# ZSHCRWY25/3DRVO-MARL-CollisionAvoidance

Hardware: AMD Instinct MI355X
Metric: drone-steps/sec (env.step throughput) (higher is better)
Workload: dtype f64; 1 GPU; BASELINE config 3 env.step: 64 drones x 4096 envs per GPU, nm=10, 0 buildings, map [50.0, 50.0, 10.0], fused step+auto-reset, f32 actions in HBM; envs_per_gpu=4096, drones=64, diag_build=False, cold_all=False, ablate=0, device_error_word=0

## Files before the change

### 3drvo-marl-collisionavoidance_amd/csrc/rvo3d_capi.hip

```cpp
#include "../../include/rvo3d.h"
#include "rvo3d_device.hpp"

#include <atomic>
#include <cmath>
#include <cstdio>
#include <cstdlib>
#include <cstring>
#include <exception>
#include <new>
#include <string>
#include <vector>

using rvo3d::Params;

namespace {
thread_local std::string g_err;

int fail(int code, const std::string& msg) {
  g_err = msg;
  return code;
}
#define HIP_TRY(expr)                                                            \
  do {                                                                           \
    hipError_t _e = (expr);                                                      \
// ... 197 lines not shown
int launch_policy_rnn_tiles(const rvo3d::RnnTilesArgs& A, unsigned grid, hipStream_t s) {
  constexpr int lds = rvo3d::kRnnTilesWaves * H * 128;
  if (int rc = allow_dynamic_lds<rvo3d::policy_rnn_tiles_kernel<H, ND>>(lds)) return rc;
  hipLaunchKernelGGL((rvo3d::policy_rnn_tiles_kernel<H, ND>), dim3(grid), dim3(64 * rvo3d::kRnnTilesWaves), lds, s, A);
  HIP_TRY(hipGetLastError());
  return RVO3D_OK;
}
bool rnn_tiles_shape_ok(int32_t hidden, int32_t in_dim, int32_t state_dim) {
  return (hidden == 64 || hidden == 256) && in_dim == 9 && state_dim >= 1 && state_dim <= 16;
}

std::atomic<uint64_t*> g_step_dev{nullptr};

rvo3d::PolicySampleArgs sample_args(int32_t tanh_out, const float* log_std, float std_factor, uint64_t seed, uint64_t step,
                                    int64_t rows, float* act, float* logp, float* val, float* dbg_mu, float* dbg_raw) {
  rvo3d::PolicySampleArgs S{};
  S.tanh_out = tanh_out; S.log_std = log_std; S.std_factor = std_factor; S.seed = seed; S.step = step;
  S.step_dev = g_step_dev.load();
  S.rows = rows; S.act = act; S.logp = logp; S.val = val; S.dbg_mu = dbg_mu; S.dbg_raw = dbg_raw;
  return S;
}

template <class Args>
int copy_reader(Args& A, const rvo3d_rnn_policy& net) {
  if (!net.w_ih_f || !net.w_hh_f || !net.b_ih_f || !net.b_hh_f || !net.ln_w || !net.ln_b)
    return fail(RVO3D_ERR_INVALID, "null reader weight");
  const bool bi = net.w_ih_r != nullptr;
  if (bi != (net.w_hh_r != nullptr) || bi != (net.b_ih_r != nullptr) || bi != (net.b_hh_r != nullptr))
    return fail(RVO3D_ERR_INVALID, "the reverse direction needs all four of w_ih_r / w_hh_r / b_ih_r / b_hh_r");
  A.w_ih[0] = net.w_ih_f; A.w_hh[0] = net.w_hh_f; A.b_ih[0] = net.b_ih_f; A.b_hh[0] = net.b_hh_f;
  A.w_ih[1] = net.w_ih_r; A.w_hh[1] = net.w_hh_r; A.b_ih[1] = net.b_ih_r; A.b_hh[1] = net.b_hh_r;
  A.ln_w = net.ln_w; A.ln_b = net.ln_b; A.eps = net.ln_eps;
  return RVO3D_OK;
}
template <class Args>
int copy_heads(Args& A, const rvo3d_mlp_weights& pi, const rvo3d_mlp_weights& v, const char* missing) {
  const rvo3d_mlp_weights* n[2] = {&pi, &v};
  for (int i = 0; i < 2; ++i) {
    if (!n[i]->w1 || !n[i]->b1 || !n[i]->w2 || !n[i]->b2 || !n[i]->w3 || !n[i]->b3)
      return fail(RVO3D_ERR_INVALID, missing);
    A.w1[i] = n[i]->w1; A.b1[i] = n[i]->b1; A.w2[i] = n[i]->w2; A.b2[i] = n[i]->b2; A.w3[i] = n[i]->w3; A.b3[i] = n[i]->b3;
  }
  return RVO3D_OK;
}

template <bool X3>
int64_t mlp_net_bytes(int ks1) { return X3 ? rvo3d::mlp_x3_net_bytes(ks1) : rvo3d::mlp_net_bytes(ks1); }

template <bool X3>
int64_t policy_mlp_blob_bytes(int32_t obs_width) {
  if (obs_width < 1 || obs_width > 126) return -1;
  return 2 * mlp_net_bytes<X3>(rvo3d::mlp_ks1(obs_width));
}

template <bool X3>
int policy_mlp_pack(const rvo3d_mlp_weights* pi, const rvo3d_mlp_weights* v, int32_t obs_width, void* blob, void* stream) {
  if (!pi || !v || !blob) return fail(RVO3D_ERR_INVALID, "null pointer");
  if (obs_width < 1 || obs_width > 126) return fail(RVO3D_ERR_INVALID, "obs_width must be 1..126");
  if (reinterpret_cast<uintptr_t>(blob) & 15) return fail(RVO3D_ERR_INVALID, "blob must be 16-byte aligned");
  rvo3d::MlpPackArgs A;
  A.k_in = obs_width; A.ks1 = rvo3d::mlp_ks1(obs_width);
  if (int rc = copy_heads(A, *pi, *v, "null weight pointer")) return rc;
  A.blob = static_cast<unsigned char*>(blob);
  hipLaunchKernelGGL(X3 ? rvo3d::mlp_x3_pack_kernel : rvo3d::mlp_pack_kernel, dim3(64, 2), dim3(256), 0,
                     static_cast<hipStream_t>(stream), A);
  HIP_TRY(hipGetLastError());
  return RVO3D_OK;
}

template <bool X3>
int policy_mlp_sample(const void* blob, int32_t obs_width, const float* obs, int64_t obs_ld, int64_t rows,
                      const int32_t* vo_count, int32_t state_dim, int32_t row_dim, int32_t tanh_out, const float* log_std,
                      float std_factor, uint64_t seed, uint64_t step, float* act, float* logp, float* val, float* dbg_mu,
                      float* dbg_raw, void* stream) {
  if (!blob || !obs || !log_std || !act || !logp || !val) return fail(RVO3D_ERR_INVALID, "null pointer");
  if (obs_width < 1 || obs_width > 126) return fail(RVO3D_ERR_INVALID, "obs_width must be 1..126");
  if (rows < 0 || obs_ld < obs_width) return fail(RVO3D_ERR_INVALID, "rows < 0 or obs_ld < obs_width");
  if (rows > 0 && ((rows - 1) * obs_ld + obs_width) * 4 > (int64_t)0x7fffffff)
    return fail(RVO3D_ERR_INVALID, "the observation array must stay below 2 GiB per call (32-bit buffer offsets): split the rows");
  if (reinterpret_cast<uintptr_t>(obs) & 3) return fail(RVO3D_ERR_INVALID, "obs must be 4-byte aligned");
  if (reinterpret_cast<uintptr_t>(blob) & 15) return fail(RVO3D_ERR_INVALID, "blob must be 16-byte aligned");
  if (rows == 0) return RVO3D_OK;
  int dev = 0, cus = 0;
  HIP_TRY(hipGetDevice(&dev));
  HIP_TRY(hipDeviceGetAttribute(&cus, hipDeviceAttributeMultiprocessorCount, dev));
  const int ks1 = rvo3d::mlp_ks1(obs_width);
  rvo3d::PolicyMlpArgs A;
  A.blob = static_cast<const unsigned char*>(blob); A.net_bytes = mlp_net_bytes<X3>(ks1);
  A.obs = obs; A.ld_obs = obs_ld; A.k_in = obs_width;
  A.cnt = vo_count; A.state_dim = state_dim; A.row_dim = row_dim;
  if (vo_count && (state_dim < 0 || row_dim < 1 || state_dim > obs_width))
    return fail(RVO3D_ERR_INVALID, "vo_count needs 0 <= state_dim <= obs_width and row_dim >= 1");
  A.S = sample_args(tanh_out, log_std, std_factor, seed, step, rows, act, logp, val, dbg_mu, dbg_raw);
  const int64_t nchunks = (rows + 63) / 64;
  int64_t G = (nchunks + kMlpWaves - 1) / kMlpWaves;
  const int64_t Gmax = cus >= 2 ? cus / 2 : 1;
  if (G > Gmax) G = Gmax;
  const unsigned grid = (unsigned)(2 * G);
  hipStream_t s = static_cast<hipStream_t>(stream);
  switch (ks1) {
    case 1: return launch_policy_mlp<X3, 1>(A, grid, s);
    case 2: return launch_policy_mlp<X3, 2>(A, grid, s);
    case 3: return launch_policy_mlp<X3, 3>(A, grid, s);
    case 4: return launch_policy_mlp<X3, 4>(A, grid, s);
    case 5: return launch_policy_mlp<X3, 5>(A, grid, s);
    case 6: return launch_policy_mlp<X3, 6>(A, grid, s);
    case 7: return launch_policy_mlp<X3, 7>(A, grid, s);
    default: return launch_policy_mlp<X3, 8>(A, grid, s);
  }
}
}

extern "C" {

int rvo3d_version(void) { return RVO3D_VERSION; }
const char* rvo3d_last_error(void) { return g_err.c_str(); }

int rvo3d_create(const rvo3d_config* cfg, rvo3d_env** out) {
  RVO3D_API_BEGIN
  if (!cfg || !out) return fail(RVO3D_ERR_INVALID, "null argument");
  *out = nullptr;
  if (cfg->num_envs < 1 || cfg->num_drones < 1 || cfg->num_drones > rvo3d::kMaxThreads)
    return fail(RVO3D_ERR_INVALID, "need num_envs >= 1 and 1 <= num_drones <= 512");
  if (cfg->max_points < 2 || cfg->num_buildings < 0 || cfg->neighbors_num < 0)
    return fail(RVO3D_ERR_INVALID, "need max_points >= 2, num_buildings >= 0, neighbors_num >= 0");
  if ((long long)cfg->num_envs * cfg->num_drones > (1ll << 30))
    return fail(RVO3D_ERR_INVALID, "num_envs * num_drones too large");
  if (cfg->action_decimals > 9) return fail(RVO3D_ERR_INVALID, "action_decimals must be <= 9");
  DeviceGuard dg;
  if (int rc0 = dg.enter(cfg->device)) return rc0;

  rvo3d_env* h = new (std::nothrow) rvo3d_env();
  if (!h) return fail(RVO3D_ERR_INVALID, "out of host memory");
  struct Owner {
    rvo3d_env* p;
    ~Owner() {
      if (!p) return;
      if (p->arena) (void)hipFree(p->arena);
      delete p;
    }
  } owner{h};
  h->cfg = *cfg;
  Params& P = h->P;
  rvo3d::Cold& C = h->cold;
  std::memset(&P, 0, sizeof P);
  std::memset(&C, 0, sizeof C);
  P.E = cfg->num_envs; P.N = cfg->num_drones; P.P = cfg->max_points;
  C.nb = cfg->num_buildings; P.nm = cfg->neighbors_num; P.env_train = cfg->env_train ? 1 : 0;
  P.W = 12 + 9 * P.nm;
#ifdef RVO3D_DIAG
  if (const char* ab = std::getenv("RVO3D_ABLATE")) P.ablate = std::atoi(ab);
#endif
  C.act_scale = cfg->action_decimals >= 0 ? std::pow(10.0, cfg->action_decimals) : 0.0;
  for (int k = 0; k < 3; ++k) C.map[k] = cfg->map_size[k];
  P.T10 = sq_threshold(10.0);
  C.T5 = sq_threshold(5.0);
  C.bgx = C.bgy = 0; C.bg_inv = 0.0;
  if (cfg->num_buildings > 0 && cfg->map_size[0] > 0 && cfg->map_size[1] > 0 &&
      std::isfinite(cfg->map_size[0]) && std::isfinite(cfg->map_size[1])) {
    const double cs = std::fmax(8.0, std::fmax(cfg->map_size[0], cfg->map_size[1]) / 64.0);
    C.bgx = (int)std::ceil(cfg->map_size[0] / cs); C.bgy = (int)std::ceil(cfg->map_size[1] / cs);
    if (C.bgx < 1) C.bgx = 1;
    if (C.bgy < 1) C.bgy = 1;
    C.bg_inv = 1.0 / cs;
  }
  C.T04 = sq_threshold(0.4);
  {
    double mx = std::fmax(C.map[0], std::fmax(C.map[1], C.map[2]));
    if (!(mx > 0)) mx = 1.0;
    for (int k = 0; k < 3; ++k) C.cen[k] = 0.5 * C.map[k];
    const double cmax = 0.75 * mx + 16.0;
    const double u = std::ldexp(1.0, -24);
    const double eD = u * (2.0 * cmax + 21.0);
    const double band = 2.0 * (2.0 * 1.7320508 * 10.5 * eD + 3.0 * eD * eD + 8.0 * u * 110.25);
    C.cmax = (float)cmax;
    P.band = std::nextafter((float)band, INFINITY);
    const float t10f = std::nextafter((float)(P.T10 + band), INFINITY);
    P.t10n = -std::nextafter(t10f, INFINITY);
    P.bandn = P.band + P.t10n;
    C.kdot = std::nextafter((float)(2.0 * (eD + 4.0 * u * 10.5) * 1.001), INFINITY);
    const double gap = 512.0 * band;
    const double cs = 4.0 * (1.7320508 * eD / std::sqrt(gap) + 8.0 * u);
    P.x1_gap = (float)gap;
    P.x1_k2 = (float)(1.0 - (4e-3 + 4.0 * cs));
    const double cs_out = cs > 1e-3 ? cs : 1e-3;
    P.x1_cs2 = (float)(cs_out * cs_out);
  }

  const int N = P.N;
  int nw = (N + 63) / 64;
  P.nw = nw <= 4 ? nw : 8;
  int epb = P.nw == 1 ? 64 / N : 1;
  if (epb > P.E) epb = P.E;
  const int ring = (P.nw >= 2 && P.nw <= 4) ? 64 * P.nw : N;
  const int threads = P.nw == 1 ? 64 : (int)align_up((size_t)ring, 64);
  size_t lds = rvo3d::lds_bytes(threads, P.nm, epb, ring, P.nw);
#ifdef RVO3D_DIAG
  if (const char* pad = std::getenv("RVO3D_LDS_PAD")) lds += (size_t)std::atoi(pad);
#endif
  if (lds > 160 * 1024) {
    return fail(RVO3D_ERR_INVALID, "neighbors_num * num_drones needs more than 160 KiB of LDS");
  }
  P.epb = epb;
  C.zf_div = (uint32_t)((P.W & 1) == 0 ? (P.W - 12) / 2 : (P.W - 12));
  C.zf_magic = 0;
  if (C.zf_div > 0) {
    const uint32_t m = (uint32_t)(((1ull << 32) + C.zf_div - 1) / C.zf_div);
    bool ok = true;
    const uint64_t qmax = (uint64_t)threads * C.zf_div;
    for (uint64_t q = 0; q < qmax && ok; ++q) ok = ((q * m) >> 32) == q / C.zf_div;
    if (!ok) {
      return fail(RVO3D_ERR_INVALID, "neighbors_num too large for the zero-fill index trick");
    }
    C.zf_magic = m;
  }
  C.zf_q = (P.W & 1) == 0 ? (uint32_t)(P.W / 2) : 0u;
  C.zf_iters = 0;
  static_assert(rvo3d::kMaxThreads / 4 <= sizeof(C.zmask) / sizeof(C.zmask[0]),
                "Cold::zmask has one word per thread quad of the largest workgroup");
  std::memset(C.zmask, 0, sizeof C.zmask);
  {
    const uint32_t rb = 4u * (uint32_t)P.W;
    const uint32_t rows_full = (uint32_t)epb * (uint32_t)N, nwv = (uint32_t)threads / 64u;
    const uint32_t nblk = rows_full * rb >> 6;
    const uint32_t iters = (nblk + 16u * nwv - 1u) / (16u * nwv);
    if (C.zf_q != 0 && P.W >= 48 && (rows_full & 7u) == 0 && iters <= 32u) {
      for (uint32_t tq = 0; tq < (uint32_t)threads / 4u; ++tq) {
        uint32_t m = 0;
        for (uint32_t i = 0; i < iters; ++i) {
          const uint32_t blk = tq + 16u * nwv * i;
          if (blk >= nblk) break;
          const uint32_t o = (blk * 64u) % rb;
          if (o >= 48u && o + 64u <= rb) m |= 1u << i;
        }
        C.zmask[tq] = m;
      }
      C.zf_iters = (int)iters;
    }
  }
  h->threads = threads;
  h->blocks = (P.E + epb - 1) / epb;
  h->lds = (int)lds;
  if (lds > 64 * 1024) {
    const bool ok = P.nw == 1 ? allow_lds_all<1>((int)lds) : (P.nw == 8 && allow_lds_all<8>((int)lds));
    if (!ok) {
      return fail(RVO3D_ERR_HIP, "hipFuncSetAttribute(MaxDynamicSharedMemorySize) failed");
    }
  }
  int rc = carve(h);
  if (rc != RVO3D_OK) return rc;
  owner.p = nullptr;
  *out = h;
  return RVO3D_OK;
  RVO3D_API_END
}

int rvo3d_destroy(rvo3d_env* h) {
  RVO3D_API_BEGIN
  if (!h) return RVO3D_OK;
  DeviceGuard dg;
  (void)dg.enter(h->cfg.device);
  (void)hipDeviceSynchronize();
  if (h->arena) (void)hipFree(h->arena);
  delete h;
  return RVO3D_OK;
  RVO3D_API_END
}

int rvo3d_load_world(rvo3d_env* h, const double* waypoints, const int32_t* n_points,
                     const double* buildings, const double* radius, const double* priority,
                     void* stream) {
  RVO3D_API_BEGIN
  DeviceGuard dg;
  int rc = check(h, false, dg);
  if (rc) return rc;
  if (!waypoints || !n_points) return fail(RVO3D_ERR_INVALID, "waypoints / n_points are required");
  const Params& P = h->P;
  const rvo3d::Cold& C = h->cold;
  if (C.nb > 0 && !buildings) return fail(RVO3D_ERR_INVALID, "buildings required when num_buildings > 0");
  hipStream_t s = static_cast<hipStream_t>(stream);
  const size_t EN = (size_t)P.E * P.N;
  std::vector<double> wp((size_t)P.P * 3 * EN), rl(EN), rad(EN), pri(EN), p95(P.P);
  for (size_t g = 0; g < EN; ++g) {
    const int np = n_points[g];
    if (np < 2 || np > P.P) return fail(RVO3D_ERR_INVALID, "n_points entries must be in [2, max_points]");
    const double* src = waypoints + g * P.P * 3;
    double total = 0.0;
    for (int k = 0; k < P.P; ++k) {
      const int kk = k < np ? k : np - 1;
      for (int c = 0; c < 3; ++c) wp[((size_t)k * 3 + c) * EN + g] = src[kk * 3 + c];
      if (k + 1 < np) {
        const double dx = src[(k + 1) * 3] - src[k * 3], dy = src[(k + 1) * 3 + 1] - src[k * 3 + 1],
                     dz = src[(k + 1) * 3 + 2] - src[k * 3 + 2];
        total += std::sqrt(py_sq(dx) + py_sq(dy) + py_sq(dz));
      }
    }
    rl[g] = total;
    rad[g] = radius ? radius[g] : 0.2;
    pri[g] = priority ? priority[g] : 5.0;
  }
  {
    bool uni = true;
    for (size_t g = 1; g < EN && uni; ++g)
      uni = std::memcmp(&rad[g], &rad[0], 8) == 0 && std::memcmp(&pri[g], &pri[0], 8) == 0;
    h->P.uniform_rp = uni ? 1 : 0;
    h->P.r0 = rad[0];
// ... 586 lines not shown
```

### 3drvo-marl-collisionavoidance_amd/csrc/rvo3d_math.hpp

```cpp
#pragma once

#include "rvo3d_params.hpp"

namespace rvo3d {

__device__ __forceinline__ double sq(double x) { return x * x; }
__device__ __forceinline__ double dot3b(double ax, double ay, double az, double bx,
                                        double by, double bz) {
  return __builtin_fma(az, bz, __builtin_fma(ay, by, ax * bx));
}
__device__ __forceinline__ double norm3b(double x, double y, double z) {
  return __builtin_sqrt(dot3b(x, y, z, x, y, z));
}
__device__ __forceinline__ double norm2sq(double x, double y) { return __builtin_fma(y, y, x * x); }
__device__ __forceinline__ bool finite_d(double q) { return __builtin_fabs(q) < __builtin_inf(); }

__device__ __forceinline__ float round2_f32(double x) {
  const double k = __builtin_rint(x * 100.0);
  return __builtin_fabs(k) < 16777216.0 ? (float)(k * 0.01) : (float)(k / 100.0);
}
__device__ __forceinline__ double k_over_1000(double k) {
  const double q = k * 0.001;
  const double r = __builtin_fma(-q, 1000.0, k);
  const double c = q + r * 0.001;
  return finite_d(k) ? c : k;
}

constexpr uint32_t kDvInvalid = 0xffffffffu;
__device__ __forceinline__ void dv_encode(const double dv[3], uint32_t& a, uint32_t& b) {
  const double k0 = __builtin_rint(dv[0] * 1000.0), k1 = __builtin_rint(dv[1] * 1000.0),
               k2 = __builtin_rint(dv[2] * 1000.0);
  const bool ok = __builtin_fabs(k0) <= 1023.0 && __builtin_fabs(k1) <= 1023.0 &&
                  __builtin_fabs(k2) <= 1023.0 && k_over_1000(k0) == dv[0] &&
                  k_over_1000(k1) == dv[1] && k_over_1000(k2) == dv[2];
  const uint32_t nz = (uint32_t)(k0 == 0.0 && __builtin_signbit(dv[0])) |
                      ((uint32_t)(k1 == 0.0 && __builtin_signbit(dv[1])) << 1) |
                      ((uint32_t)(k2 == 0.0 && __builtin_signbit(dv[2])) << 2);
  a = ok ? ((uint32_t)((int)k0 + 1024) | ((uint32_t)((int)k1 + 1024) << 16)) : kDvInvalid;
  b = (uint32_t)((int)(ok ? k2 : 0.0) + 1024) | (nz << 16);
}
__device__ __forceinline__ bool dv_decode(uint32_t a, uint32_t b, double dv[3]) {
  if (a == kDvInvalid) return false;
  const int k0 = (int)(a & 0xffffu) - 1024, k1 = (int)(a >> 16) - 1024, k2 = (int)(b & 0xffffu) - 1024;
  dv[0] = (b & (1u << 16)) ? -0.0 : k_over_1000((double)k0);
  dv[1] = (b & (1u << 17)) ? -0.0 : k_over_1000((double)k1);
  dv[2] = (b & (1u << 18)) ? -0.0 : k_over_1000((double)k2);
  return true;
}

__device__ __forceinline__ double py_round2_c(double x) {
  double p = x * 100.0;
  double e = __builtin_fma(x, 100.0, -p);
  double c = __builtin_floor(p);
  double d = (p - (c + 0.5)) + e;
  if (d > 0.0) c += 1.0;
  else if (d == 0.0 && (((long long)c) & 1)) c += 1.0;
  return c;
}
__device__ __forceinline__ double clampd(double x, double lo, double hi) {
  return x < lo ? lo : (x > hi ? hi : x);
}
__device__ __forceinline__ double np_mod(double a, double b) {
  double m;
  if (b > 0.0 && a > -b && a < 2.0 * b) m = a >= b ? a - b : a;
  else m = fmod(a, b);
  if (m != 0.0) {
    if ((b < 0.0) != (m < 0.0)) m += b;
  } else {
    m = __builtin_copysign(0.0, b);
  }
  return m;
}

__device__ __forceinline__ void des_vel(const Params& P, const double p[3], const double cur[3],
                                        double out[3]) {
  const double dx = cur[0] - p[0], dy = cur[1] - p[1], dz = cur[2] - p[2];
  const double d2 = dot3b(dx, dy, dz, dx, dy, dz);
  if (d2 > P.cold().T04) {
    const double inv = 1000.0 / __builtin_sqrt(d2);
    const double ux = dx * inv, uy = dy * inv, uz = dz * inv;
    double kx = __builtin_rint(ux), ky = __builtin_rint(uy), kz = __builtin_rint(uz);
    const double m = __builtin_fmin(__builtin_fmin(0.5 - __builtin_fabs(ux - kx),
                                                   0.5 - __builtin_fabs(uy - ky)),
                                    0.5 - __builtin_fabs(uz - kz));
    if (!(m > 1e-7)) {
      const double az = atan2(dy, dx);
      const double el = atan2(dz, __builtin_sqrt(norm2sq(dx, dy)));
      double sa, ca, se, ce;
      sincos(az, &sa, &ca);
      sincos(el, &se, &ce);
      kx = __builtin_rint((1.0 * (ca * ce)) * 1000.0);
      ky = __builtin_rint((1.0 * (sa * ce)) * 1000.0);
      kz = __builtin_rint((1.0 * se) * 1000.0);
    }
    out[0] = k_over_1000(kx); out[1] = k_over_1000(ky); out[2] = k_over_1000(kz);
  } else {
    out[0] = out[1] = out[2] = 0.0;
  }
}

__device__ __forceinline__ double deviation(const double a[3], const double b[3],
                                            const double p[3]) {
  double dx = b[0] - a[0], dy = b[1] - a[1], dz = b[2] - a[2];
  double mag = __builtin_sqrt(sq(dx) + sq(dy) + sq(dz));
  if (mag == 0.0) return 0.0;
  double hx = dx / mag, hy = dy / mag, hz = dz / mag;
  double qx0 = p[0] - a[0], qy0 = p[1] - a[1], qz0 = p[2] - a[2];
  double t = qx0 * hx + qy0 * hy + qz0 * hz;
  double qx = a[0] + t * hx, qy = a[1] + t * hy, qz = a[2] + t * hz;
  return __builtin_sqrt(sq(p[0] - qx) + sq(p[1] - qy) + sq(p[2] - qz));
}

__device__ __forceinline__ bool arrived(const Params& P, const double p[3], const double d[3]) {
  const double x = p[0] - d[0], y = p[1] - d[1], z = p[2] - d[2];
  return dot3b(x, y, z, x, y, z) <= P.cold().T04;
}

__device__ __forceinline__ double vo_exp_time(double rx, double ry, double rz, double rvx,
                                              double rvy, double rvz, double ra, double rb) {
  double r = ra + rb;
  double ux = -rvx, uy = -rvy, uz = -rvz;
  double a = sq(ux) + sq(uy) + sq(uz);
  double b = 2 * rx * ux + 2 * ry * uy + 2 * rz * uz;
  double c = sq(rx) + sq(ry) + sq(rz) - sq(r);
  if (c <= 0) return 0.0;
  double temp = sq(b) - 4 * a * c;
  if (temp <= 0) return __builtin_inf();
  double s = __builtin_sqrt(temp);
  double t1 = (-b + s) / (2 * a);
  double t2 = (-b - s) / (2 * a);
  if (t1 < 0 && t2 < 0) return -1.0;
  double t3 = t1 >= 0 ? t1 : __builtin_inf();
  double t4 = t2 >= 0 ? t2 : __builtin_inf();
  return t4 < t3 ? t4 : t3;
}

struct Drone {
  double x, y, z, vx, vy, vz, r, prio;
};

struct PairOut {
  bool collision, flag;
  double t, iet, md;
  int alpha_c;
};

}
```

### 3drvo-marl-collisionavoidance_amd/csrc/rvo3d_params.hpp

```cpp
#pragma once

#include <hip/hip_runtime.h>
#include <stdint.h>

namespace rvo3d {

constexpr double kExpRadius = 0.2;
constexpr double kCtimeThreshold = 2.0;
constexpr double kDeg2Rad = 0.017453292519943295;
constexpr double kPi = 3.141592653589793;
constexpr int kMaxThreads = 512;
constexpr double kCosD = 0.999999995;
constexpr double kSinD = 1.0000000000e-4;

struct Cold {
  double map[3];
  double T5, T04;
  double cen[3];
  double act_scale;
  float cmax;
  float kdot;
  uint32_t zf_div;
  uint32_t zf_magic;
  uint32_t zf_q;
  int zf_iters;
  uint32_t zmask[128];
  int nb;
  const double* bld;
  const double* pow95;
  const uint16_t* bgrid;
  int bgx, bgy;
  double bg_inv;
};
constexpr int kBgridK = 15;
typedef const __attribute__((address_space(4))) Cold ColdC;

struct Params {
  int E, N, P, nm, env_train, epb, W;
  int action_f64;
  int dv_cached;
  int g_cached;
  int action_mode;
  float acceler;
#ifdef RVO3D_DIAG
  int ablate;
#endif
  int zf16;
  int uniform_rp;
  double r0, prio0;
  double T10;
  float t10n;
  float bandn;
  float band;
  int nw;
  float x1_gap;
  float x1_k2;
  float x1_cs2;
  double* f64;
  int32_t* i32;
  uint8_t* u8;
  uint32_t S;
  enum { F_PX, F_PY, F_PZ, F_VX, F_VY, F_VZ, F_YAW, F_PITCH, F_REAL_LEN, F_MAX_DEV, F_EXTRA_LEN,
         F_CUR, F_PREV = F_CUR + 3,
         F_ROUTE_LEN = F_PREV + 3, F_RADIUS, F_PRIO, F_DEV0, F_WP };
  __host__ __device__ double* f(int k) const { return f64 + (size_t)k * S; }
  __host__ __device__ double* px() const { return f(F_PX); }
  __host__ __device__ double* py() const { return f(F_PY); }
  __host__ __device__ double* pz() const { return f(F_PZ); }
  __host__ __device__ double* vx() const { return f(F_VX); }
  __host__ __device__ double* vy() const { return f(F_VY); }
  __host__ __device__ double* vz() const { return f(F_VZ); }
  __host__ __device__ double* yaw() const { return f(F_YAW); }
  __host__ __device__ double* pitch() const { return f(F_PITCH); }
  __host__ __device__ double* real_len() const { return f(F_REAL_LEN); }
  __host__ __device__ double* max_dev() const { return f(F_MAX_DEV); }
  __host__ __device__ double* extra_len() const { return f(F_EXTRA_LEN); }
  __host__ __device__ int32_t* wp_idx() const { return i32; }
  __host__ __device__ uint8_t* arrive() const { return u8; }
  __host__ __device__ uint8_t* dest() const { return u8 + S; }
  __host__ __device__ double* route_len() const { return f(F_ROUTE_LEN); }
  __host__ __device__ double* radius() const { return f(F_RADIUS); }
  __host__ __device__ double* prio() const { return f(F_PRIO); }
  __host__ __device__ double* dev0() const { return f(F_DEV0); }
  __host__ __device__ double* wp(int k, int c) const { return f(F_WP + 3 * k + c); }
  __host__ __device__ double* cur(int c) const { return f(F_CUR + c); }
  __host__ __device__ double* prev(int c) const { return f(F_PREV + c); }
  __host__ __device__ int32_t* n_points() const { return i32 + S; }
  __host__ __device__ uint32_t* dvk_a() const { return reinterpret_cast<uint32_t*>(i32) + (size_t)2 * S; }
  __host__ __device__ uint32_t* dvk_b() const { return reinterpret_cast<uint32_t*>(i32) + (size_t)3 * S; }
  __host__ __device__ uint32_t* dv0_a() const { return reinterpret_cast<uint32_t*>(i32) + (size_t)4 * S; }
  __host__ __device__ uint32_t* dv0_b() const { return reinterpret_cast<uint32_t*>(i32) + (size_t)5 * S; }
  __host__ __device__ uint32_t* gcache(int w) const { return reinterpret_cast<uint32_t*>(i32) + (size_t)(6 + w) * S; }
  __host__ __device__ double* row_iet(int s) const { return f(F_WP + 3 * P + s); }
  __host__ __device__ uint32_t* row_pk(int s) const {
    return reinterpret_cast<uint32_t*>(i32) + (size_t)(6 + nw + s) * S;
  }
  __host__ __device__ static size_t f64_arrays(int P_, int nm_) { return F_WP + 3 * (size_t)P_ + (nm_ > 0 ? nm_ : 1); }
  __host__ __device__ static size_t i32_arrays(int nm_, int nw_) { return 6 + (size_t)nw_ + (size_t)(nm_ > 0 ? nm_ : 1); }
  uint32_t* err;
  const Cold* cold_;
  __device__ __forceinline__ ColdC& cold() const { return *(ColdC*)cold_; }
#ifdef RVO3D_DIAG
  unsigned long long* dbg;
#endif
  const void* actions;
  float* obs;
  int32_t* vo_count;
  float* reward;
  double* reward64;
  uint8_t *done, *info, *finish, *reset_mask;
  const int32_t* prev_cnt;
};

#ifdef RVO3D_DIAG
#define RVO3D_STAMP(i)                                                                  \
  do {                                                                                  \
    if (P.dbg && threadIdx.x == 0) P.dbg[(size_t)blockIdx.x * 32 + (i)] = __builtin_amdgcn_s_memtime(); \
  } while (0)
#define RVO3D_ABLATED(bits) ((P.ablate & (bits)) != 0)
#else
#define RVO3D_STAMP(i) do { } while (0)
#define RVO3D_ABLATED(bits) false
#endif

}
```

### 3drvo-marl-collisionavoidance_amd/csrc/rvo3d_step.hpp

```cpp
#pragma once

#include "rvo3d_pairs.hpp"

namespace rvo3d {

__device__ __forceinline__ bool building_test(const double* const bld, int b, const Drone& S,
                                              double T5) {
  const double bx = bld[4 * b], by = bld[4 * b + 1], bh = bld[4 * b + 2], br = bld[4 * b + 3];
  const double ex = S.x - bx, ey = S.y - by;
  if ((bh > S.z - 2) & (norm2sq(ex, ey) <= T5) & (S.z <= bh))
    return __builtin_sqrt(sq(ex) + sq(ey)) <= S.r + br;
  return false;
}
__device__ __forceinline__ bool building_hit(const Params& P, const Drone& S) {
  const int nb = P.cold().nb;
  if (nb == 0) return false;
  bool hit = false;
  const double* const bld = P.cold().bld;
  const double T5 = P.cold().T5;
  const int gx = P.cold().bgx;
  if (gx > 0) {
    const int gy = P.cold().bgy;
    const double inv = P.cold().bg_inv;
    int ix = (int)__builtin_floor(S.x * inv), iy = (int)__builtin_floor(S.y * inv);
// ... 267 lines not shown
}
__device__ __forceinline__ void store3(double* const a0, double* const a1, double* const a2, int g,
                                       const double v[3]) {
  a0[g] = v[0]; a1[g] = v[1]; a2[g] = v[2];
}
#define RVO3D_LOAD_CUR(P, g, out) load3((P).cur(0), (P).cur(1), (P).cur(2), g, out)
#define RVO3D_LOAD_PREV(P, g, out) load3((P).prev(0), (P).prev(1), (P).prev(2), g, out)
#define RVO3D_STORE_CUR(P, g, v) store3((P).cur(0), (P).cur(1), (P).cur(2), g, v)
#define RVO3D_STORE_PREV(P, g, v) store3((P).prev(0), (P).prev(1), (P).prev(2), g, v)

__device__ __forceinline__ double rvo_reward_pre(const double dv[3], const double a[3]) {
  const double d0 = dv[0], d1 = dv[1], d2 = dv[2];
  const double vel_penalty = 0.2 * norm3b(a[0], a[1], a[2]) / norm3b(d0, d1, d2);
  const double eps = 1e-8;
  const double magA = __builtin_sqrt(sq(d0) + sq(d1) + sq(d2) + eps);
  const double magB = __builtin_sqrt(sq(a[0]) + sq(a[1]) + sq(a[2]) + eps);
  const double dotp = d0 * a[0] + d1 * a[1] + d2 * a[2];
  double c = dotp / (magA * magB);
  c = c < -1.0 + eps ? -1.0 + eps : (c > 1.0 - eps ? 1.0 - eps : c);
  const double C18 = 0.984807753012208, C6 = 0.8660254037844387, C3 = 0.5000000000000001,
               C2 = 6.123233995736766e-17;
  double punish;
  if (c == 0.0) punish = -4;
  else if (__builtin_fabs(c - C18) > 1e-12 && __builtin_fabs(c - C6) > 1e-12 &&
           __builtin_fabs(c - C3) > 1e-12 && __builtin_fabs(c - C2) > 1e-12) {
    punish = c > C18 ? 3 : (c > C6 ? 1 : (c > C3 ? 0.5 : (c > C2 ? 0 : -4)));
    if (c != c) punish = -4;
  } else {
    const double ang = acos(c);
    if (ang < kPi / 18) punish = 3;
    else if (ang < kPi / 6) punish = 1;
    else if (ang < kPi / 3) punish = 0.5;
    else if (ang < kPi / 2) punish = 0;
    else punish = -4;
  }
  return punish + vel_penalty;
}
__device__ __forceinline__ double rvo_reward_k(double pre, bool flag, double tmin) {
  double safety = 0;
  if (flag) {
    double urgency = 0;
    if (tmin < 2) urgency = -8.0 * exp(-tmin / 0.5);
    safety = -2.5 + urgency;
  }
  return __builtin_rint((pre + safety) * 1000.0);
}

__device__ __forceinline__ double mov_reward_k(const Params& P, bool collision, bool arrive_r,
                                               int waypoint_num, int n_points_m1, bool dest_r,
                                               double dev, bool len_flag, double exlen) {
  if (collision) return -50000.0;
  double reward = 0;
  if (arrive_r) reward += 3.0 * P.cold().pow95[n_points_m1 - waypoint_num];
  if (dest_r) reward += 20.0;
  const double d = dev * 10;
  const double dev_pen = -1.5 * (2 / (1 + exp(-(d - 5) / 0.3)));
  double ex_pen = 0;
  if (len_flag) {
    ex_pen = -0.3 * log(exlen + 1 + 1e-6);
    if (ex_pen < -6 || ex_pen != ex_pen) ex_pen = -6;
  }
  return __builtin_rint((reward + dev_pen + ex_pen) * 1000.0);
}


enum Mode { kObserve = 0, kStep = 1, kStepAutoReset = 2 };

#ifndef RVO3D_ZERO_NT
#define RVO3D_ZERO_NT 1
#endif
#ifndef RVO3D_DEPHASE
#define RVO3D_DEPHASE 0
#endif

#ifndef RVO3D_WAVES_ATTR
#define RVO3D_WAVES_ATTR __attribute__((amdgpu_waves_per_eu(NW <= 4 ? 4 : 3)))
#endif

template <int MODE, int NW, int NFIX = 0, bool TRAIN = true, bool PAD = (NFIX != 0 && NW > 1)>
__global__ void __launch_bounds__(64 * NW) RVO3D_WAVES_ATTR env_kernel(const Params Pin) {
  extern __shared__ __attribute__((aligned(16))) unsigned char smem[];
  Params P = Pin;
  static_assert(!PAD || NFIX != 0, "a padded kernel has a compile-time ring size");
  const int Nr = Pin.N;
  if (NFIX) { P.N = NFIX; P.epb = NFIX <= 64 ? 64 / NFIX : 1; }
  const int tid = threadIdx.x, T = (NW == 1 || NFIX) ? 64 * NW : (int)blockDim.x, N = P.N;
  const Lds L = carve_lds(smem, T, P.nm, P.epb, N, NW);
  const int el = tid / N;
  const int d = tid - el * N;
  const int e0 = blockIdx.x * P.epb;
  const int e = e0 + el;
  const bool active = (el < P.epb) && (e < P.E) && (!PAD || d < Nr);
  const int g = active ? e * (PAD ? Nr : N) + d : 0;
  const int lbase = el * N;
  const int full_rows = P.epb * (PAD ? Nr : N);
  const int nrows = ((P.E - e0) < P.epb ? (P.E - e0) : P.epb) * (PAD ? Nr : N);
  const int row0 = e0 * (PAD ? Nr : N);
  const int lrow = PAD ? el * Nr + d : tid;
  constexpr bool LITE = (MODE == kStepAutoReset);
  constexpr bool GSH = NW > 1 && NFIX == 64 * NW;
  constexpr bool XQ = NW == 1 && NFIX != 0;

  RVO3D_STAMP(0);
#if RVO3D_DEPHASE
  if (NW == 1) {
    unsigned hw_slot;
    asm volatile("s_getreg_b32 %0, hwreg(HW_REG_HW_ID)" : "=s"(hw_slot));
    if (hw_slot & 1)
      for (int i = 0; i < RVO3D_DEPHASE; ++i) __builtin_amdgcn_s_sleep(32);
  }
#endif
  Drone S;
  S.x = S.y = S.z = S.vx = S.vy = S.vz = 0.0; S.r = 0.2; S.prio = 5;
  if (PAD && d >= Nr) {
    S.x = S.y = S.z = __builtin_inf();
    const int o = el * 2 * N + d, os = el * N + d;
#pragma unroll
    for (int k = 0; k < 12; ++k) {
      const float v = (k == WX || k == WY || k == WZ) ? 1e30f : (k == WKD ? -1.0f : 0.0f);
      if (k == WX || k == WY || k == WZ || k == WR) {
        L.w[k][o] = v;
        if (d <= (N >> 1)) L.w[k][o + N] = v;
      } else L.w[k][os] = v;
    }
  }
  double a[3] = {0, 0, 0}, cur[3] = {0, 0, 0}, dv[3] = {0, 0, 0};
  double dev = 0, max_dev = 0;
  int wpi = 1;

  uint32_t gw[NW];
  const bool have_gw = MODE != kObserve && P.g_cached != 0;
  uint32_t old_cnt = 0;
  if (active) {
    if (LITE && NW == 1 && P.prev_cnt) {
      old_cnt = (uint32_t)P.prev_cnt[g];
      old_cnt = old_cnt < (uint32_t)P.nm ? old_cnt : (uint32_t)P.nm;
    }
    S.x = P.px()[g]; S.y = P.py()[g]; S.z = P.pz()[g];
    S.vx = P.vx()[g]; S.vy = P.vy()[g]; S.vz = P.vz()[g];
    if (P.uniform_rp) { S.r = P.r0; S.prio = P.prio0; }
    else { S.r = P.radius()[g]; S.prio = P.prio()[g]; }
    if (have_gw) {
#pragma unroll
      for (int w = 0; w < NW; ++w) gw[w] = P.gcache(w)[g];
    }
    if (MODE != kObserve) {
      if (P.action_mode == 1) {
        const float* A = static_cast<const float*>(P.actions) + (size_t)g * 3;
        const double vv[3] = {S.vx, S.vy, S.vz};
#pragma unroll
        for (int k = 0; k < 3; ++k) {
          const float r = __builtin_rintf(A[k] * 100.0f) / 100.0f;
          const double x = (double)(P.acceler * r) + vv[k];
          a[k] = __builtin_rint(x * 100.0) / 100.0;
        }
      } else {
        if (P.action_f64) {
          const double* A = static_cast<const double*>(P.actions) + (size_t)g * 3;
          a[0] = A[0]; a[1] = A[1]; a[2] = A[2];
        } else {
          const float* A = static_cast<const float*>(P.actions) + (size_t)g * 3;
          a[0] = (double)A[0]; a[1] = (double)A[1]; a[2] = (double)A[2];
        }
        if (P.cold().act_scale > 0) {
          a[0] = __builtin_rint(a[0] * P.cold().act_scale) / P.cold().act_scale;
          a[1] = __builtin_rint(a[1] * P.cold().act_scale) / P.cold().act_scale;
          a[2] = __builtin_rint(a[2] * P.cold().act_scale) / P.cold().act_scale;
        }
      }
    }
  }
  RVO3D_STAMP(1);
  double az[3] = {a[0], a[1], a[2]};
  if (norm3b(a[0], a[1], a[2]) < 1e-5) az[0] = az[1] = az[2] = 0.0;
  const double zero3[3] = {0, 0, 0};

  if (tid < P.epb) { L.any_reset[tid] = 0; L.far[tid] = 0; }
  if (LITE && NW > 1 && tid == 0) *L.any_old = 0;
  L.kept[tid] = 0;
  __syncthreads();
  if (LITE && NW == 1 && active && P.prev_cnt) L.kept[lrow] = (int)old_cnt;
  L.x[tid] = S.x; L.y[tid] = S.y; L.z[tid] = S.z;
  L.vx[tid] = S.vx; L.vy[tid] = S.vy; L.vz[tid] = S.vz;
  L.r[tid] = S.r; L.prio[tid] = S.prio;
  {
    const double p[3] = {S.x, S.y, S.z}, v[3] = {S.vx, S.vy, S.vz};
    stage_f32<NW>(P, L, el, d, active, p, v, az, S.r, S.prio);
  }
  __syncthreads();

  bool flag, collision = false;
  double tmin;

  if (MODE == kObserve) {
    if (active) {
      double prev[3];
      max_dev = P.max_dev()[g];
      RVO3D_LOAD_CUR(P, g, cur);
      RVO3D_LOAD_PREV(P, g, prev);
      const double p[3] = {S.x, S.y, S.z};
      des_vel(P, p, cur, dv);
      dev = deviation(prev, cur, p);
      if (dev > max_dev) max_dev = dev;
    }
    const int kept = sweep_env<NW, true, true, TRAIN, GSH, XQ>(P, L, tid, el, d, g, active, S, zero3, true, true, flag,
                                               tmin, collision, gw, false);
    if (active) {
      write_vo_rows(P, L, tid, lbase, g, S, kept);
      if (P.zf16) stage_row(P, L, lrow, g, S, proprio_tail(dv, dev), kept);
      else {
        write_proprio(P, g, S, proprio_tail(dv, dev));
        publish_zero_run(P, g, kept);
        L.kept[lrow] = kept;
      }
      P.max_dev()[g] = max_dev;
      uint32_t dvk_a, dvk_b;
      dv_encode(dv, dvk_a, dvk_b);
      P.dvk_a()[g] = dvk_a; P.dvk_b()[g] = dvk_b;
#pragma unroll
      for (int w = 0; w < NW; ++w) P.gcache(w)[g] = gw[w];
    }
    __syncthreads();
    if (P.zf16) row_fill_pairs<NW>(P, L, tid, row0, nrows);
    else zero_fill(P, L, tid, row0, nrows);
    return;
  }

  RVO3D_STAMP(2);
  sweep_env<NW, false, false, TRAIN, GSH, XQ>(P, L, tid, el, d, g, active && !RVO3D_ABLATED(1), S, az, false, false, flag,
                              tmin, collision, gw, have_gw);
  double rew_k = 0;
  double mov_nc = 0;
  bool f_dest = false;
  RVO3D_STAMP(3);
  constexpr bool kLoadAhead = NW <= 2;
  double prev[3] = {0, 0, 0}, yaw = 0, pitch = 0, real_len = 0, route_len = 0;
  int npts = 2;
  bool f_arrive_in = false, f_dest_in = false;
#define RVO3D_LOAD_INTEGRATION_STATE()                                               \
  {                                                                                  \
    wpi = P.wp_idx()[g];                                                             \
    RVO3D_LOAD_PREV(P, g, prev);                                                     \
    yaw = P.yaw()[g]; pitch = P.pitch()[g]; real_len = P.real_len()[g];              \
    route_len = P.route_len()[g];                                                    \
    npts = P.n_points()[g];                                                          \
    f_arrive_in = P.arrive()[g] != 0; f_dest_in = P.dest()[g] != 0;                  \
  }
  if (active) {
    max_dev = P.max_dev()[g];
    RVO3D_LOAD_CUR(P, g, cur);
    uint32_t dvk_a = 0, dvk_b = 0;
    if (P.dv_cached) { dvk_a = P.dvk_a()[g]; dvk_b = P.dvk_b()[g]; }
    if (kLoadAhead) RVO3D_LOAD_INTEGRATION_STATE()
    bool have = false;
    if (P.dv_cached) have = dv_decode(dvk_a, dvk_b, dv);
    if (!have) {
      if (!kLoadAhead) RVO3D_LOAD_PREV(P, g, prev);
      const double p[3] = {S.x, S.y, S.z};
      des_vel(P, p, cur, dv);
      dev = deviation(prev, cur, p);
      if (dev > max_dev) max_dev = dev;
    }
    rew_k = rvo_reward_k(rvo_reward_pre(dv, a), flag, tmin);
  }
  RVO3D_STAMP(18);
  __syncthreads();
  if (active) {
    if (!kLoadAhead) RVO3D_LOAD_INTEGRATION_STATE()
#undef RVO3D_LOAD_INTEGRATION_STATE
    bool ex_set = false;
    double extra_len = 0.0;
    const int wpi_in = wpi;
    bool f_arrive = f_arrive_in;
    f_dest = f_dest_in;

    double speed = norm3b(S.vx, S.vy, S.vz);
    const double acc = clampd(a[0] * 1.0, -1.0, 1.0);
    const double dyaw = clampd(a[1] * 90.0, -90.0, 90.0);
    const double dpit = clampd(a[2] * 90.0, -90.0, 90.0);
    const double nv = speed + acc;
    speed = (0.0 > nv) ? 0.0 : nv;
    yaw = np_mod(yaw + dyaw, 360.0);
    pitch = clampd(pitch + dpit, -90.0, 90.0);
    double nvx = 0.0, nvy = 0.0, nvz = 0.0;
    if (!f_dest) {
      double sy, cy, sp, cp;
      sincos(yaw * kDeg2Rad, &sy, &cy);
      sincos(pitch * kDeg2Rad, &sp, &cp);
      nvx = speed * cp * cy; nvy = speed * cp * sy; nvz = speed * sp;
    }
    const double q0 = S.x, q1 = S.y, q2 = S.z;
    S.x = S.x + nvx; S.y = S.y + nvy; S.z = S.z + nvz;
    S.vx = nvx; S.vy = nvy; S.vz = nvz;
    real_len = real_len + norm3b(S.x - q0, S.y - q1, S.z - q2);
    const double p[3] = {S.x, S.y, S.z};
    double dst[3] = {0, 0, 0};
    if (f_arrive || arrived(P, p, cur)) load_wp(P, g, npts - 1, dst);
    if (arrived(P, p, cur)) {
      const bool at_dst = arrived(P, p, dst);
      if (at_dst) { extra_len = real_len - route_len; ex_set = true; }
      if (!at_dst && wpi < npts - 1) {
        wpi += 1;
        prev[0] = cur[0]; prev[1] = cur[1]; prev[2] = cur[2];
        load_wp(P, g, wpi, cur);
        RVO3D_STORE_CUR(P, g, cur);
        RVO3D_STORE_PREV(P, g, prev);
        f_arrive = false;
      }
    }
    des_vel(P, p, cur, dv);
    dev = deviation(prev, cur, p);
    if (dev > max_dev) max_dev = dev;
    bool arrive_r = false, dest_r = false;
    const int waypoint_num = wpi;
    if (!f_arrive && arrived(P, p, cur)) { f_arrive = true; arrive_r = true; }
    if (f_arrive) {
      if (arrived(P, p, dst)) {
        extra_len = real_len - route_len;
        ex_set = true;
        if (!f_dest) { f_dest = true; dest_r = true; }
      }
    }
    const double exlen = real_len - route_len + 4;
    mov_nc = mov_reward_k(P, false, arrive_r, waypoint_num, npts - 1, dest_r, dev, exlen > 0,
                          exlen);
    RVO3D_STAMP(19);
    collision = building_hit(P, S);
    if (S.x < 0 || S.x > P.cold().map[0] || S.y < 0 || S.y > P.cold().map[1] || S.z < 0 || S.z > P.cold().map[2])
      collision = true;
    P.yaw()[g] = yaw; P.pitch()[g] = pitch; P.real_len()[g] = real_len;
    if (ex_set) P.extra_len()[g] = extra_len;
    if (wpi != wpi_in) P.wp_idx()[g] = wpi;
    if (f_arrive != f_arrive_in) P.arrive()[g] = f_arrive ? 1 : 0;
    if (f_dest != f_dest_in) P.dest()[g] = f_dest ? 1 : 0;
    P.info[g] = f_arrive ? 1 : 0;
    P.finish[g] = f_dest ? 1 : 0;
  }
  L.x[tid] = S.x; L.y[tid] = S.y; L.z[tid] = S.z;
  L.vx[tid] = S.vx; L.vy[tid] = S.vy; L.vz[tid] = S.vz;
  {
    const double p[3] = {S.x, S.y, S.z}, v[3] = {S.vx, S.vy, S.vz};
    stage_f32<NW>(P, L, el, d, active, p, v, az, S.r, S.prio);
  }
  __syncthreads();

  RVO3D_STAMP(4);
  int kept = 0;
  if (LITE) {
    if (collide_env<NW, TRAIN, GSH>(P, L, tid, el, d, active && !RVO3D_ABLATED(2), S, gw)) collision = true;
  } else {
    kept = sweep_env<NW, true, true, TRAIN, GSH, XQ>(P, L, tid, el, d, g, active && !RVO3D_ABLATED(2), S, az, false,
                                     false, flag, tmin, collision, gw, false);
  }
  bool do_reset = false;
  if (active) {
    const double rew64 = k_over_1000(rew_k) + k_over_1000(collision ? -50000.0 : mov_nc);
    P.reward[g] = (float)rew64;
    if (P.reward64) P.reward64[g] = rew64;
    P.done[g] = collision ? 1 : 0;
    do_reset = LITE && (collision || f_dest);
  }

  RVO3D_STAMP(5);
  if (LITE) {
    if (active && P.reset_mask) P.reset_mask[g] = do_reset ? 1 : 0;
    if (do_reset) L.any_reset[el] = 1;
    __syncthreads();
    double p[3] = {0, 0, 0}, rcur[3] = {0, 0, 0}, rdev = 0.0;
    uint32_t rdv_a = 0, rdv_b = 0;
    if (NW > 1 && active && P.prev_cnt) {
      old_cnt = (uint32_t)P.prev_cnt[g];
      old_cnt = old_cnt < (uint32_t)P.nm ? old_cnt : (uint32_t)P.nm;
      L.kept[lrow] = (int)old_cnt;
      if (old_cnt != 0) *L.any_old = 1;
    }
    if (do_reset) {
      load_wp(P, g, 0, p);
      rdev = P.dev0()[g];
      load_wp(P, g, 1, rcur);
      rdv_a = P.dv0_a()[g]; rdv_b = P.dv0_b()[g];
    }
    RVO3D_STAMP(26);
    if (NW == 1 && two_phase_rows(P, row0, nrows, full_rows) && !RVO3D_ABLATED(16)) early_zero_blocks<NW>(P, L, tid, row0, nrows);
    RVO3D_STAMP(27);
    if (do_reset) {
      S.x = p[0]; S.y = p[1]; S.z = p[2]; S.vx = S.vy = S.vz = 0.0;
      dev = rdev;
      cur[0] = rcur[0]; cur[1] = rcur[1]; cur[2] = rcur[2];
      if (!dv_decode(rdv_a, rdv_b, dv)) {
        des_vel(P, p, cur, dv);
        dev = deviation(p, cur, p);
      }
      RVO3D_STORE_CUR(P, g, cur);
      RVO3D_STORE_PREV(P, g, p);
      max_dev = dev > 0.0 ? dev : 0.0;
      P.wp_idx()[g] = 1; P.arrive()[g] = 0; P.dest()[g] = 0;
      P.real_len()[g] = 0.0; P.yaw()[g] = 0.0; P.pitch()[g] = 0.0;
      L.x[tid] = S.x; L.y[tid] = S.y; L.z[tid] = S.z;
      L.vx[tid] = 0.0; L.vy[tid] = 0.0; L.vz[tid] = 0.0;
      const double v0[3] = {0, 0, 0};
      stage_f32<NW>(P, L, el, d, true, p, v0, az, S.r, S.prio);
    }
    if (active && L.any_reset[el] != 0) {
      const int os = el * N + d;
      L.w[WAX][os] = 0.f; L.w[WAY][os] = 0.f; L.w[WAZ][os] = 0.f;
    }
  }
  if (active) {
    uint32_t dvk_a, dvk_b;
    dv_encode(dv, dvk_a, dvk_b);
    P.dvk_a()[g] = dvk_a; P.dvk_b()[g] = dvk_b;
  }
  const ProprioTail ptail = proprio_tail(dv, dev);
  if (active) P.max_dev()[g] = max_dev;
  if (LITE) {
    __syncthreads();
    RVO3D_STAMP(6);
    const bool env_reset = (active || (PAD && el < P.epb)) && (L.any_reset[el] != 0);
    bool c2 = false;
    const double aa[3] = {env_reset ? 0.0 : az[0], env_reset ? 0.0 : az[1], env_reset ? 0.0 : az[2]};
    bool have_gw2 = !env_reset;
    if (NW == 1) {
      const unsigned long long rlanes = __ballot(do_reset);
      if (L.far[el] != 0) {
        uint32_t valid[1];
        valid_offsets<1>(N, d, valid);
        gw[0] = valid[0];
      } else {
        gw[0] = regate_resets(P, L, tid, el, d, active, rlanes, gw[0]);
      }
      have_gw2 = true;
    }
    if (RVO3D_ABLATED(2)) have_gw2 = false;
    if (NW > 1 && two_phase_rows(P, row0, nrows, full_rows) && !RVO3D_ABLATED(16)) early_zero_blocks<NW>(P, L, tid, row0, nrows);
    kept = sweep_env<NW, true, false, TRAIN, GSH, XQ>(P, L, tid, el, d, g, active && !RVO3D_ABLATED(4), S, aa,
                                      false, env_reset, flag, tmin, c2, gw, have_gw2);
  }
  RVO3D_STAMP(7);
  const bool two_phase = LITE && two_phase_rows(P, row0, nrows, full_rows);
  if (NW > 1 && two_phase) {
    asm volatile("s_waitcnt vmcnt(0)" ::: "memory");
    __syncthreads();
  }
  if (active) {
    if (!RVO3D_ABLATED(8)) {
      if (two_phase) asm volatile("s_waitcnt vmcnt(0)" ::: "memory");
      write_vo_rows(P, L, tid, lbase, g, S, kept);
      RVO3D_STAMP(16);
      if (P.zf16) stage_row(P, L, lrow, g, S, ptail, kept);
      else { write_proprio(P, g, S, ptail); publish_zero_run(P, g, kept); }
    }
    if (!P.zf16) L.kept[lrow] = kept;
  }
  __syncthreads();
  RVO3D_STAMP(17);
  if (!RVO3D_ABLATED(16)) {
    if (two_phase) late_row_windows<NW>(P, L, tid, row0, nrows);
    else if (P.zf16) row_fill_pairs<NW>(P, L, tid, row0, nrows);
    else zero_fill(P, L, tid, row0, nrows);
  }
  RVO3D_STAMP(8);
  if (active) {
#pragma unroll
    for (int w = 0; w < NW; ++w) P.gcache(w)[g] = gw[w];
    P.px()[g] = S.x; P.py()[g] = S.y; P.pz()[g] = S.z;
    P.vx()[g] = S.vx; P.vy()[g] = S.vy; P.vz()[g] = S.vz;
  }
  RVO3D_STAMP(9);
}

}
```

Baseline: 7.764 billion drone-steps/s.

## Hoist reset-state loads before collision sweep and replace action rounding divisions

```diff
diff --git a/3drvo-marl-collisionavoidance_amd/csrc/rvo3d_capi.hip b/3drvo-marl-collisionavoidance_amd/csrc/rvo3d_capi.hip
--- a/3drvo-marl-collisionavoidance_amd/csrc/rvo3d_capi.hip
+++ b/3drvo-marl-collisionavoidance_amd/csrc/rvo3d_capi.hip
@@ -373,6 +373,7 @@
   if (const char* ab = std::getenv("RVO3D_ABLATE")) P.ablate = std::atoi(ab);
 #endif
   C.act_scale = cfg->action_decimals >= 0 ? std::pow(10.0, cfg->action_decimals) : 0.0;
+  C.act_inv = (C.act_scale == 10.0 || C.act_scale == 100.0 || C.act_scale == 1000.0) ? 1.0 / C.act_scale : 0.0;
   for (int k = 0; k < 3; ++k) C.map[k] = cfg->map_size[k];
   P.T10 = sq_threshold(10.0);
   C.T5 = sq_threshold(5.0);
diff --git a/3drvo-marl-collisionavoidance_amd/csrc/rvo3d_math.hpp b/3drvo-marl-collisionavoidance_amd/csrc/rvo3d_math.hpp
--- a/3drvo-marl-collisionavoidance_amd/csrc/rvo3d_math.hpp
+++ b/3drvo-marl-collisionavoidance_amd/csrc/rvo3d_math.hpp
@@ -24,6 +24,13 @@
   const double r = __builtin_fma(-q, 1000.0, k);
   const double c = q + r * 0.001;
   return finite_d(k) ? c : k;
+}
+__device__ __forceinline__ double k_over_scale(double k, double s, double inv) {
+  if (inv == 0.0 || !(__builtin_fabs(k) < 9007199254740992.0)) return k / s;
+  const double q = k * inv;
+  const double r = __builtin_fma(-q, s, k);
+  const double c = __builtin_fma(r, inv, q);
+  return k == 0.0 ? k : c;
 }
 
 constexpr uint32_t kDvInvalid = 0xffffffffu;
diff --git a/3drvo-marl-collisionavoidance_amd/csrc/rvo3d_params.hpp b/3drvo-marl-collisionavoidance_amd/csrc/rvo3d_params.hpp
--- a/3drvo-marl-collisionavoidance_amd/csrc/rvo3d_params.hpp
+++ b/3drvo-marl-collisionavoidance_amd/csrc/rvo3d_params.hpp
@@ -18,6 +18,7 @@
   double T5, T04;
   double cen[3];
   double act_scale;
+  double act_inv;
   float cmax;
   float kdot;
   uint32_t zf_div;
diff --git a/3drvo-marl-collisionavoidance_amd/csrc/rvo3d_step.hpp b/3drvo-marl-collisionavoidance_amd/csrc/rvo3d_step.hpp
--- a/3drvo-marl-collisionavoidance_amd/csrc/rvo3d_step.hpp
+++ b/3drvo-marl-collisionavoidance_amd/csrc/rvo3d_step.hpp
@@ -443,7 +443,7 @@
         for (int k = 0; k < 3; ++k) {
           const float r = __builtin_rintf(A[k] * 100.0f) / 100.0f;
           const double x = (double)(P.acceler * r) + vv[k];
-          a[k] = __builtin_rint(x * 100.0) / 100.0;
+          a[k] = k_over_scale(__builtin_rint(x * 100.0), 100.0, 0.01);
         }
       } else {
         if (P.action_f64) {
@@ -454,9 +454,10 @@
           a[0] = (double)A[0]; a[1] = (double)A[1]; a[2] = (double)A[2];
         }
         if (P.cold().act_scale > 0) {
-          a[0] = __builtin_rint(a[0] * P.cold().act_scale) / P.cold().act_scale;
-          a[1] = __builtin_rint(a[1] * P.cold().act_scale) / P.cold().act_scale;
-          a[2] = __builtin_rint(a[2] * P.cold().act_scale) / P.cold().act_scale;
+          const double s = P.cold().act_scale, inv = P.cold().act_inv;
+          a[0] = k_over_scale(__builtin_rint(a[0] * s), s, inv);
+          a[1] = k_over_scale(__builtin_rint(a[1] * s), s, inv);
+          a[2] = k_over_scale(__builtin_rint(a[2] * s), s, inv);
         }
       }
     }
@@ -555,6 +556,17 @@
     rew_k = rvo_reward_k(rvo_reward_pre(dv, a), flag, tmin);
   }
   RVO3D_STAMP(18);
+  constexpr bool kEarlyReset = LITE && NW == 1;
+  bool early = false;
+  double rp[3] = {0, 0, 0};
+  uint32_t rdv_a = 0, rdv_b = 0;
+#define RVO3D_LOAD_RESET_STATE()                                                     \
+  {                                                                                  \
+    load_wp(P, g, 0, rp);                                                            \
+    dev = P.dev0()[g];                                                               \
+    load_wp(P, g, 1, cur);                                                           \
+    rdv_a = P.dv0_a()[g]; rdv_b = P.dv0_b()[g];                                      \
+  }
   __syncthreads();
   if (active) {
     if (!kLoadAhead) RVO3D_LOAD_INTEGRATION_STATE()
@@ -619,11 +631,15 @@
     collision = building_hit(P, S);
     if (S.x < 0 || S.x > P.cold().map[0] || S.y < 0 || S.y > P.cold().map[1] || S.z < 0 || S.z > P.cold().map[2])
       collision = true;
-    P.yaw()[g] = yaw; P.pitch()[g] = pitch; P.real_len()[g] = real_len;
+    if (kEarlyReset) {
+      early = collision || f_dest;
+      if (early) RVO3D_LOAD_RESET_STATE()
+    }
+    P.yaw()[g] = early ? 0.0 : yaw; P.pitch()[g] = early ? 0.0 : pitch; P.real_len()[g] = early ? 0.0 : real_len;
     if (ex_set) P.extra_len()[g] = extra_len;
-    if (wpi != wpi_in) P.wp_idx()[g] = wpi;
-    if (f_arrive != f_arrive_in) P.arrive()[g] = f_arrive ? 1 : 0;
-    if (f_dest != f_dest_in) P.dest()[g] = f_dest ? 1 : 0;
+    if (early ? wpi_in != 1 : wpi != wpi_in) P.wp_idx()[g] = early ? 1 : wpi;
+    if (early ? f_arrive_in : f_arrive != f_arrive_in) P.arrive()[g] = (f_arrive && !early) ? 1 : 0;
+    if (early ? f_dest_in : f_dest != f_dest_in) P.dest()[g] = (f_dest && !early) ? 1 : 0;
     P.info[g] = f_arrive ? 1 : 0;
     P.finish[g] = f_dest ? 1 : 0;
   }
@@ -644,59 +660,66 @@
                                      false, flag, tmin, collision, gw, false);
   }
   bool do_reset = false;
+  double rew64 = 0.0;
   if (active) {
-    const double rew64 = k_over_1000(rew_k) + k_over_1000(collision ? -50000.0 : mov_nc);
-    P.reward[g] = (float)rew64;
-    if (P.reward64) P.reward64[g] = rew64;
-    P.done[g] = collision ? 1 : 0;
+    rew64 = k_over_1000(rew_k) + k_over_1000(collision ? -50000.0 : mov_nc);
     do_reset = LITE && (collision || f_dest);
   }
+#define RVO3D_STORE_STEP_RESULT()                                                    \
+  if (active) {                                                                      \
+    P.reward[g] = (float)rew64;                                                      \
+    if (P.reward64) P.reward64[g] = rew64;                                           \
+    P.done[g] = collision ? 1 : 0;                                                   \
+    if (LITE && P.reset_mask) P.reset_mask[g] = do_reset ? 1 : 0;                    \
+  }
+  if (!kEarlyReset) RVO3D_STORE_STEP_RESULT()
 
   RVO3D_STAMP(5);
   if (LITE) {
-    if (active && P.reset_mask) P.reset_mask[g] = do_reset ? 1 : 0;
     if (do_reset) L.any_reset[el] = 1;
     __syncthreads();
-    double p[3] = {0, 0, 0}, rcur[3] = {0, 0, 0}, rdev = 0.0;
-    uint32_t rdv_a = 0, rdv_b = 0;
+    const bool late = do_reset && !early;
+    const bool any_late = !kEarlyReset || __ballot(late) != 0ull;
     if (NW > 1 && active && P.prev_cnt) {
       old_cnt = (uint32_t)P.prev_cnt[g];
       old_cnt = old_cnt < (uint32_t)P.nm ? old_cnt : (uint32_t)P.nm;
       L.kept[lrow] = (int)old_cnt;
       if (old_cnt != 0) *L.any_old = 1;
     }
-    if (do_reset) {
-      load_wp(P, g, 0, p);
-      rdev = P.dev0()[g];
-      load_wp(P, g, 1, rcur);
-      rdv_a = P.dv0_a()[g]; rdv_b = P.dv0_b()[g];
-    }
+    if (any_late) {
+      if (late) RVO3D_LOAD_RESET_STATE()
+    }
+#undef RVO3D_LOAD_RESET_STATE
     RVO3D_STAMP(26);
     if (NW == 1 && two_phase_rows(P, row0, nrows, full_rows) && !RVO3D_ABLATED(16)) early_zero_blocks<NW>(P, L, tid, row0, nrows);
     RVO3D_STAMP(27);
     if (do_reset) {
-      S.x = p[0]; S.y = p[1]; S.z = p[2]; S.vx = S.vy = S.vz = 0.0;
-      dev = rdev;
-      cur[0] = rcur[0]; cur[1] = rcur[1]; cur[2] = rcur[2];
+      S.x = rp[0]; S.y = rp[1]; S.z = rp[2]; S.vx = S.vy = S.vz = 0.0;
       if (!dv_decode(rdv_a, rdv_b, dv)) {
-        des_vel(P, p, cur, dv);
-        dev = deviation(p, cur, p);
+        des_vel(P, rp, cur, dv);
+        dev = deviation(rp, cur, rp);
       }
       RVO3D_STORE_CUR(P, g, cur);
-      RVO3D_STORE_PREV(P, g, p);
+      RVO3D_STORE_PREV(P, g, rp);
       max_dev = dev > 0.0 ? dev : 0.0;
-      P.wp_idx()[g] = 1; P.arrive()[g] = 0; P.dest()[g] = 0;
-      P.real_len()[g] = 0.0; P.yaw()[g] = 0.0; P.pitch()[g] = 0.0;
+      if (any_late) {
+        if (late) {
+          P.wp_idx()[g] = 1; P.arrive()[g] = 0; P.dest()[g] = 0;
+          P.real_len()[g] = 0.0; P.yaw()[g] = 0.0; P.pitch()[g] = 0.0;
+        }
+      }
       L.x[tid] = S.x; L.y[tid] = S.y; L.z[tid] = S.z;
       L.vx[tid] = 0.0; L.vy[tid] = 0.0; L.vz[tid] = 0.0;
       const double v0[3] = {0, 0, 0};
-      stage_f32<NW>(P, L, el, d, true, p, v0, az, S.r, S.prio);
+      stage_f32<NW>(P, L, el, d, true, rp, v0, az, S.r, S.prio);
     }
     if (active && L.any_reset[el] != 0) {
       const int os = el * N + d;
       L.w[WAX][os] = 0.f; L.w[WAY][os] = 0.f; L.w[WAZ][os] = 0.f;
     }
-  }
+    if (kEarlyReset) RVO3D_STORE_STEP_RESULT()
+  }
+#undef RVO3D_STORE_STEP_RESULT
   if (active) {
     uint32_t dvk_a, dvk_b;
     dv_encode(dv, dvk_a, dvk_b);
```

Result: no change. 7.835 billion drone-steps/s (median of 6 runs) (+0.9%).
